# ArielleRosinski/pyGAT

Hardware: AMD Instinct MI355X
Metric: GAT-layer fwd+bwd edges/sec (higher is better)
Workload: dtype f32; 1 GPU; RMAT scale 20 (1048576 nodes, 10760610 edges incl. self loops, max degree 26737), Fin 128, 8 heads x 16, concat+ELU, dropout 0, fwd+bwd (dW, da); nodes=1048576, edges=10760610, fin=128, heads=8, f_out=16, parallelism=single GPU, heads_per_gpu=8, gemm_products=split-bf16, launch=stream launches (pygat_amd.GATLevelFn)

## Files before the change

include/pygat_amd.h:

```cpp
#ifndef PYGAT_AMD_H
#define PYGAT_AMD_H

#include <stdint.h>
#include <stddef.h>

#ifdef __cplusplus
extern "C" {
#endif

#define PYGAT_ABI_VERSION 16

enum {
  PYGAT_OK = 0,
  PYGAT_EINVAL = -1,
  PYGAT_EHIP = -2,
  PYGAT_ENODEV = -3
};

enum {
  PYGAT_F_ELU = 1,
  PYGAT_F_SKIP = 2,
  PYGAT_F_MAIN_ONLY = 4,
  PYGAT_F_FIXUP_ONLY = 8
};
// ... 31 lines not shown
                   const pygat_out_segments* out, int accumulate,
                   int split_k, void* ws, int gemm_mode, void* stream);

typedef struct {
  int w;
  int64_t stride;
} pygat_col_blocks;
int pygat_gemm_f32_blocked(int transA, int transB, int M, int N, int64_t K,
                           const float* A, int64_t lda, const pygat_col_blocks* a_blk, const float* B, int64_t ldb,
                           const pygat_out_segments* out, const pygat_col_blocks* c_blk, int accumulate,
                           int split_k, void* ws, int gemm_mode, void* stream);

int pygat_pack_params(int H, int Fin, int Fo, const float* W, const float* a,
                      const float* w_skip, float* Wcat, int64_t ldw, float* a_pad,
                      void* stream);
#define PYGAT_MAX_HEADS_TABLE 16
int pygat_pack_params_heads(int H, int Fin, int Fo, const float* const* W, const float* const* a,
                            const float* const* w_skip, float* Wcat, int64_t ldw, float* a_pad, void* stream);
int pygat_stack_heads(int H, int64_t nW, int nA, int64_t nS, const float* const* W, const float* const* a,
                      const float* const* w_skip, float* W_out, float* a_out, float* skip_out, void* stream);
int pygat_stack_heads_padded(int H, int64_t nW, int64_t nW_out, int nA, int64_t nS, int64_t nS_out, const float* const* W,
                             const float* const* a, const float* const* w_skip, float* W_out, float* a_out, float* skip_out,
                             void* stream);
int pygat_project(int n, int Fin, int H, int Fo, const float* X, int64_t ldx, const float* Wcat, int64_t ldw, const float* a_pad,
                  float* Wh, float* Sk, float* s, int split_k, void* ws, int gemm_mode, void* stream);
int pygat_project_blocked(int n, int Fin, int H, int Fo, const float* X, int64_t ldx, const pygat_col_blocks* x_blk,
                          const float* Wcat, int64_t ldw, const float* a_pad, float* Wh, float* Sk, float* s, int split_k,
                          void* ws, int gemm_mode, void* stream);
int pygat_attn_scores(int n, int H, int Fo, float* Wh, const float* wh_mask, const float* a_pad,
                      float* s, float* t, void* stream);
int pygat_unpack_wgrad(int H, int Fin, int Fo, const float* dWcat, int64_t ld,
                       int col_offset, float* dW, void* stream);

typedef struct {
  int n;
  int64_t nnz;
  const int32_t* rowptr;
  const int32_t* edge_rc;
  int slot_edges;
  const int32_t* slot_begin;
  const int32_t* cut_rows;
  int n_cut;
  int n_cut_wide;
  int64_t slot_first;
  int64_t slot_count;
  const int32_t* slot_meta;
  const int32_t* slot_order;
  const int32_t* user_row;
} pygat_graph;

int pygat_edge_pairs(int n, const int32_t* rowptr, const int32_t* col, int32_t* edge_rc, void* stream);

int pygat_slot_bounds(int n, int64_t nnz, const int32_t* rowptr, const int32_t* edge_rc, int slot_edges,
                      int32_t* slot_begin, void* stream);
int pygat_slot_meta(int n, int64_t nnz, const int32_t* rowptr, const int32_t* edge_rc, int slot_edges,
                    const int32_t* slot_begin, int32_t* slot_meta, void* stream);

size_t pygat_partials_bytes(int64_t nnz, int slot_edges, int H, int Fp);

int pygat_head_group(int n, int H, int Fo);

int pygat_gat_forward_phases_ok(int n, int H, int Fo);
int pygat_gat_forward(const pygat_graph* g, int H, int Fo, float alpha, int flags,
                      const float* Wh, const float* s, const float* a_pad, const float* sk,
                      const float* att_mask,
                      float* out, float* hattn, float* m, float* Z, float* aneg, float* qneg,
                      void* part, void* stream);

int pygat_head_mean(int n, int H, int Fo, const float* hattn, const float* sk,
                    float* out, void* stream);

int pygat_gat_backward_prepare(int n, int H, int Fo, int flags, int mean_mode,
                               const float* G, const float* y, const float* sk,
                               const float* s, const float* m, const float* Z,
                               float* GR, const float* aneg, const float* qneg, float alpha, float* ds,
                               int h_first, int h_count, int head_group, const int32_t* user_row, void* stream);
int pygat_gat_backward_row(const pygat_graph* g, int H, int Fo, float alpha,
                           const float* Wh, const float* a_pad, const float* GR,
                           const float* att_mask, float* ds, void* part, int h_first, int h_count, int head_group,
                           void* stream);
size_t pygat_gat_backward_col_da_bytes(const pygat_graph* gT, int H, int Fo, int head_group);
// ... 154 lines not shown
```

pygat_amd/_lib.py:

```python
from __future__ import annotations

import ctypes as C
import os

import torch

_HERE = os.path.dirname(os.path.abspath(__file__))
LIB_PATH = os.path.join(_HERE, "libpygat_amd.so")
from .config import config as _config
if _config.lib_path:
    LIB_PATH = os.path.abspath(_config.lib_path)

ABI_VERSION = 16
F_ELU = 1
F_SKIP = 2
F_MAIN_ONLY = 4
F_FIXUP_ONLY = 8

SYMBOLS = [
    "pygat_abi_version", "pygat_last_error", "pygat_padded_width", "pygat_device_count",
    "pygat_device_name", "pygat_kernel_footprint", "pygat_default_gemm_mode", "pygat_dense_row_counts", "pygat_scan_workspace_bytes",
    "pygat_exclusive_scan_i32", "pygat_dense_fill_cols", "pygat_csr_symmetric_perm",
    "pygat_gemm_workspace_bytes", "pygat_gemm_f32", "pygat_gemm_f32_blocked", "pygat_project_blocked", "pygat_wgrad_blocked", "pygat_pack_params", "pygat_pack_params_heads", "pygat_stack_heads", "pygat_stack_heads_padded", "pygat_project", "pygat_attn_scores",
    "pygat_unpack_wgrad",
# ... 1 lines not shown
    "pygat_gat_backward_prepare", "pygat_gat_backward_row", "pygat_gat_backward_col", "pygat_gat_backward_rowsum",
    "pygat_gat_backward_col_da_bytes", "pygat_a_grad_fold",
    "pygat_gat_backward_col_phases_ok", "pygat_gat_backward_col_phase", "pygat_gat_backward_col_finish",
    "pygat_agrad_workspace_bytes", "pygat_a_grad", "pygat_wgrad_workspace_bytes", "pygat_wgrad",
    "pygat_gatv2_forward", "pygat_gatv2_backward_prepare", "pygat_gatv2_workspace_bytes", "pygat_gatv2_backward",
    "pygat_gat_attention", "pygat_gatv2_attention",
    "pygat_alpha_grad_rows", "pygat_alpha_grad_cols", "pygat_alpha_grad_apply",
    "pygat_gat_edge_workspace_bytes", "pygat_gat_edge_forward", "pygat_gat_edge_alpha", "pygat_gat_edge_backward_rows",
    "pygat_gat_edge_backward_cols",
    "pygat_gat_bf16_workspace_bytes", "pygat_gat_pack_bf16", "pygat_gat_forward_bf16",
    "pygat_spmm_workspace_bytes", "pygat_spmm_forward", "pygat_spmm_grad_values",
    "pygat_dropout_mask", "pygat_dropout_mask2", "pygat_dropout_expand", "pygat_dropout_head_sum", "pygat_pack_blockdiag",
    "pygat_unpack_blockdiag",
    "pygat_headmask_supported", "pygat_dropout_bits", "pygat_project_dropout_workspace_bytes", "pygat_project_dropout",
    "pygat_wgrad_dropout_workspace_bytes",
    "pygat_wgrad_dropout", "pygat_dropout_head_sum_bits",
    "pygat_nll_workspace_bytes", "pygat_elu_logsoftmax_nll", "pygat_elu_logsoftmax_nll_backward",
    "pygat_project_sparse", "pygat_wgrad_sparse", "pygat_wgrad_sparse_workspace_bytes", "pygat_dropout_narrow", "pygat_dx_dropout", "pygat_adam_step", "pygat_bce_workspace_bytes", "pygat_bce_with_logits", "pygat_bce_with_logits_backward",
]

MAX_ADAM_TENSORS = 48
MAX_SEGMENTS = 4


class OutSegments(C.Structure):
    _fields_ = [("nseg", C.c_int), ("col_start", C.c_int32 * (MAX_SEGMENTS + 1)), ("ptr", C.c_void_p * MAX_SEGMENTS),
                ("ld", C.c_int64 * MAX_SEGMENTS)]


class ColBlocks(C.Structure):
    _fields_ = [("w", C.c_int), ("stride", C.c_int64)]


class Graph(C.Structure):
    _fields_ = [("n", C.c_int), ("nnz", C.c_int64), ("rowptr", C.c_void_p), ("edge_rc", C.c_void_p),
                ("slot_edges", C.c_int), ("slot_begin", C.c_void_p), ("cut_rows", C.c_void_p),
                ("n_cut", C.c_int), ("n_cut_wide", C.c_int), ("slot_first", C.c_int64), ("slot_count", C.c_int64),
                ("slot_meta", C.c_void_p), ("slot_order", C.c_void_p), ("user_row", C.c_void_p)]


def _load():
    if not os.path.exists(LIB_PATH):
        raise ImportError(
            f"pygat_amd: {LIB_PATH} not found. Build it with `python -c 'import __graft_entry__ as g; "
            f"g.build()'` or `make -C pygat_amd/csrc`. There is no CPU/PyTorch fallback for the hot path.")
    lib = C.CDLL(LIB_PATH)
    missing = [s for s in SYMBOLS if not hasattr(lib, s)]
    if missing:
        raise ImportError(f"pygat_amd: {LIB_PATH} lacks symbols {missing}")
    p, i, i64, f, sz = C.c_void_p, C.c_int, C.c_int64, C.c_float, C.c_size_t
    lib.pygat_abi_version.restype = i
    lib.pygat_last_error.restype = C.c_char_p
    lib.pygat_padded_width.argtypes = [i]
    lib.pygat_device_name.argtypes = [C.c_char_p, i]
    lib.pygat_kernel_footprint.argtypes = [C.c_char_p, C.POINTER(C.c_int), C.POINTER(C.c_int)]
    lib.pygat_default_gemm_mode.argtypes = []
    lib.pygat_dense_row_counts.argtypes = [p, i, i64, i, p, p]
    lib.pygat_scan_workspace_bytes.argtypes = [i64]
    lib.pygat_scan_workspace_bytes.restype = sz
    lib.pygat_exclusive_scan_i32.argtypes = [p, i64, p, p, p]
    lib.pygat_dense_fill_cols.argtypes = [p, i, i64, i, p, p, p]
    lib.pygat_csr_symmetric_perm.argtypes = [i, p, p, p, p, p]
    lib.pygat_gemm_workspace_bytes.argtypes = [i, i, i]
    lib.pygat_gemm_workspace_bytes.restype = sz
    lib.pygat_gemm_f32.argtypes = [i, i, i, i, i64, p, i64, p, i64, C.POINTER(OutSegments), i, i, p, i, p]
    CB = C.POINTER(ColBlocks)
    lib.pygat_gemm_f32_blocked.argtypes = [i, i, i, i, i64, p, i64, CB, p, i64, C.POINTER(OutSegments), CB, i, i, p, i, p]
    lib.pygat_project_blocked.argtypes = [i, i, i, i, p, i64, CB, p, i64, p, p, p, p, i, p, i, p]
    lib.pygat_wgrad_blocked.argtypes = [i, i, i, i, p, i64, CB, p, p, p, p, i, p, i, i, i, p]
    lib.pygat_pack_params.argtypes = [i, i, i, p, p, p, p, i64, p, p]
    lib.pygat_pack_params_heads.argtypes = [i, i, i, p, p, p, p, i64, p, p]
# ... 132 lines not shown
```

pygat_amd/csrc/core.hip:

```cpp
#include "common.h"
#include <string.h>

namespace pygat {
static thread_local char g_err[512] = "";

void set_error(const char* fmt, ...) {
  va_list ap;
  va_start(ap, fmt);
  vsnprintf(g_err, sizeof(g_err), fmt, ap);
  va_end(ap);
}

static const int g_default_split = [] { const char* e = getenv("PYGAT_GEMM_F32"); return (e && atoi(e) != 0) ? 0 : 1; }();
bool gemm_split(int mode) { return mode == PYGAT_GEMM_DEFAULT ? g_default_split != 0 : mode == PYGAT_GEMM_SPLIT_BF16; }
}

extern "C" int pygat_default_gemm_mode(void) { return pygat::g_default_split ? PYGAT_GEMM_SPLIT_BF16 : PYGAT_GEMM_FP32_MFMA; }

extern "C" int pygat_abi_version(void) { return PYGAT_ABI_VERSION; }
extern "C" const char* pygat_last_error(void) { return pygat::g_err; }
extern "C" int pygat_padded_width(int f_out) { return pygat::padded_width(f_out); }

namespace pygat {
int footprint_k2_headline(int* regs, int* scratch);
int footprint_k4_headline_da(int* regs, int* scratch);
int footprint_gemm_x3(int which, int* regs, int* scratch);
int footprint_k14(int which, int* regs, int* scratch);
int footprint_k15(const char* name, int* regs, int* scratch);
int footprint_k16(const char* name, int* regs, int* scratch);
int footprint_k17(const char* name, int* regs, int* scratch);
}

extern "C" int pygat_kernel_footprint(const char* kernel, int* num_regs, int* scratch_bytes) {
  PYGAT_REQUIRE(kernel && num_regs && scratch_bytes, "kernel_footprint: null argument");
  if (!strcmp(kernel, "k2_headline")) return pygat::footprint_k2_headline(num_regs, scratch_bytes);
  if (!strcmp(kernel, "k4_headline_da")) return pygat::footprint_k4_headline_da(num_regs, scratch_bytes);
  if (!strcmp(kernel, "tn_x3w")) return pygat::footprint_gemm_x3(0, num_regs, scratch_bytes);
  if (!strcmp(kernel, "x3gw")) return pygat::footprint_gemm_x3(1, num_regs, scratch_bytes);
  if (!strcmp(kernel, "k1_x3_tail")) return pygat::footprint_gemm_x3(2, num_regs, scratch_bytes);
  static const char* const k14[] = {"k14_rows_long", "k14_cols_long", "k14_rows_wave", "k14_cols_wave", "k14_apply"};
  for (int w = 0; w < 5; ++w)
    if (!strcmp(kernel, k14[w])) return pygat::footprint_k14(w, num_regs, scratch_bytes);
  if (!strncmp(kernel, "k15_", 4)) return pygat::footprint_k15(kernel, num_regs, scratch_bytes);
  if (!strncmp(kernel, "k16_", 4)) return pygat::footprint_k16(kernel, num_regs, scratch_bytes);
  if (!strncmp(kernel, "k17_", 4)) return pygat::footprint_k17(kernel, num_regs, scratch_bytes);
  pygat::set_error("kernel_footprint: unknown kernel '%s' (k2_headline, k4_headline_da, tn_x3w, x3gw, k1_x3_tail, k14_rows_long, "
                   "k14_cols_long, k14_rows_wave, k14_cols_wave, k14_apply)", kernel);
  return PYGAT_EINVAL;
}

extern "C" int pygat_device_count(void) {
  int n = 0;
  if (hipGetDeviceCount(&n) != hipSuccess) {
    (void)hipGetLastError();
    return 0;
  }
  return n;
}

extern "C" int pygat_device_name(char* host_buf, int len) {
  if (!host_buf || len <= 0) return PYGAT_EINVAL;
  int dev = 0;
  hipDeviceProp_t p;
  if (hipGetDevice(&dev) != hipSuccess || hipGetDeviceProperties(&p, dev) != hipSuccess) {
    (void)hipGetLastError();
    pygat::set_error("no HIP device");
    return PYGAT_ENODEV;
  }
  snprintf(host_buf, (size_t)len, "%s (%s)", p.name, p.gcnArchName);
  return PYGAT_OK;
}
```

pygat_amd/csrc/k2_forward.hip:

```cpp
#include "attn_common.h"

namespace pygat {

struct FwdArgs {
  GraphDev g;
  RowShape rs;
  float alpha;
  int flags;
  const float* Wh;
  int64_t ldwh;
  const float* s;
  const float* a_pad;
  const float* sk;
  const float* mask;
  float* out;
  float* hattn;
  float* m;
  float* Z;
  float* part;
  float* aneg;
  float* qneg;
};

__device__ __forceinline__ float lrelu(float z, float alpha) { return z > 0.f ? z : alpha * z; }

template <bool AUX>
__device__ __forceinline__ void fold_edge(float& m, float& z, float4& a, float& zn, float4& an, float ev, bool neg,
                                          float4 w, float mk) {
  const float d = ev - m;
  const float ex = __expf(-fabsf(d));
  const bool up = d > 0.f;
  const float sc = up ? ex : 1.f, p = up ? 1.f : ex;
  z = fmaf(z, sc, p);
  const float pm = p * mk;
  a.x = fmaf(a.x, sc, pm * w.x); a.y = fmaf(a.y, sc, pm * w.y);
  a.z = fmaf(a.z, sc, pm * w.z); a.w = fmaf(a.w, sc, pm * w.w);
  if constexpr (AUX) {
    const float pn = neg ? p : 0.f, pmn = neg ? pm : 0.f;
    zn = fmaf(zn, sc, pn);
    an.x = fmaf(an.x, sc, pmn * w.x); an.y = fmaf(an.y, sc, pmn * w.y);
    an.z = fmaf(an.z, sc, pmn * w.z); an.w = fmaf(an.w, sc, pmn * w.w);
  }
  m = up ? ev : m;
}

template <bool AUX>
__device__ __forceinline__ void merge_state(float& m, float& z, float4& a, float& zn, float4& an, float m2, float z2,
                                            float4 a2, float zn2, float4 an2) {
  const float mn = fmaxf(m, m2);
  const float sa = __expf(m - mn), sb = __expf(m2 - mn);
  z = z * sa + z2 * sb;
  a.x = a.x * sa + a2.x * sb; a.y = a.y * sa + a2.y * sb;
  a.z = a.z * sa + a2.z * sb; a.w = a.w * sa + a2.w * sb;
  if constexpr (AUX) {
// ... 82 lines not shown
    st4(p + lc.cofs[v], st.acc[v]);
    if constexpr (AUX) st4(p + R + 2 * H + lc.cofs[v], st.accn[v]);
    if (((lc.cofs[v] >> 2) & (a.rs.lph - 1)) == 0) {
      p[R + lc.head[v]] = st.m[v];
      p[R + H + lc.head[v]] = st.z[v];
      if constexpr (AUX) p[2 * R + 2 * H + lc.head[v]] = st.zn[v];
    }
  }
}
template <int VEC, bool AUX>
struct PartRec {
  float m[VEC], z[VEC];
  float4 acc[VEC];
  float zn[AUX ? VEC : 1];
  float4 accn[AUX ? VEC : 1];
};
template <int VEC, bool AUX>
__device__ __forceinline__ void part_load(const FwdArgs& a, const LaneCols<VEC>& lc, const float* p, PartRec<VEC, AUX>& r) {
  const int R = a.rs.R, H = a.rs.H;
#pragma unroll
  for (int v = 0; v < VEC; ++v) {
    r.m[v] = p[R + lc.head[v]]; r.z[v] = p[R + H + lc.head[v]]; r.acc[v] = ld4(p + lc.cofs[v]);
    if constexpr (AUX) { r.zn[v] = p[2 * R + 2 * H + lc.head[v]]; r.accn[v] = ld4(p + R + 2 * H + lc.cofs[v]); }
  }
}
template <int VEC, bool AUX>
__device__ __forceinline__ void part_merge(RowState<VEC, AUX>& st, const PartRec<VEC, AUX>& r) {
#pragma unroll
  for (int v = 0; v < VEC; ++v)
    merge_state<AUX>(st.m[v], st.z[v], st.acc[v], st.zn[AUX ? v : 0], st.accn[AUX ? v : 0], r.m[v], r.z[v], r.acc[v],
                     r.zn[AUX ? v : 0], r.accn[AUX ? v : 0]);
}

template <int LPR, int VEC, bool AUX, int LPH = 0, int CR = 0>
__device__ __forceinline__ void fwd_flush(const FwdArgs& a, const LaneCols<VEC>& lc, int64_t k, int i,
                                          bool is_head, bool is_tail, const RowState<VEC, AUX>& st) {
  if (is_head || is_tail) {
    part_store<VEC, AUX>(a, lc, a.part + (2 * k + (is_head ? 0 : 1)) * part_stride<AUX>(a.rs), st);
  } else {
    fwd_finish<LPR, VEC, AUX, LPH, CR>(a, lc, i, st);
  }
}

#ifndef PYGAT_K2_PREFETCH_ALL
#define PYGAT_K2_PREFETCH_ALL 0
#endif
#ifndef PYGAT_K2_PREFETCH_TRAIN
#define PYGAT_K2_PREFETCH_TRAIN 1
#endif
#ifndef PYGAT_K2_HEADLINE_WAVES
#define PYGAT_K2_HEADLINE_WAVES 4
#endif
#ifndef PYGAT_K2_NARROW_U
#define PYGAT_K2_NARROW_U 4
#endif
template <int LPR, int VEC, bool V2, bool AUX, bool FAST, int LPH = 0, int CR = 0>
__global__ __launch_bounds__(256) __attribute__((amdgpu_waves_per_eu((AUX && FAST && VEC == 1 && LPR > 8) ? PYGAT_K2_HEADLINE_WAVES : 1))) void gat_fwd_kernel(FwdArgs a) {
  constexpr int EPW = 64 / LPR;
  constexpr bool NARROW = (VEC == 1 && LPR <= 8);
  constexpr bool PREF = NARROW || (PYGAT_K2_PREFETCH_ALL && VEC == 1) || (PYGAT_K2_PREFETCH_TRAIN && AUX && FAST && VEC == 1);
  constexpr int U = (VEC == 1) ? (NARROW ? PYGAT_K2_NARROW_U : 4) : 2;
  const int lane = threadIdx.x & 63;
  const int64_t kl = ((int64_t)blockIdx.x * (blockDim.x >> 6) + (threadIdx.x >> 6)) * EPW + lane / LPR;
  if (kl >= a.g.kn) return;
  const int64_t k = a.g.order ? a.g.order[kl] : a.g.k0 + kl;
  int64_t e0, e1;
  const int2* __restrict__ rc = a.g.rc;
  int r_first;
  bool head_partial, tail_known = false, tail_flag = false;
  if (a.g.meta) {
    const int4 mt = a.g.meta[k];
    e0 = mt.x; e1 = mt.y; r_first = mt.z;
    head_partial = (mt.w & 1) != 0; tail_known = true; tail_flag = (mt.w & 2) != 0;
  } else {
    slot_range(a.g, k, &e0, &e1);
    r_first = rc[e0].x;
    head_partial = a.g.rowptr[r_first] < e0;
  }
  const LaneCols<VEC> lc = lane_cols<LPR, VEC>(a.rs);
  const int R = CR ? CR : a.rs.R;
  const int64_t ldh = CR ? CR / (4 * (LPH ? LPH : 1)) : a.rs.ldh;

  int cur = r_first;
  const int lph = LPH > 0 ? LPH : (a.rs.lph < 64 ? a.rs.lph : 64);
  float4 adst[VEC];
#pragma unroll
  for (int v = 0; v < VEC; ++v) {
    adst[v] = V2 ? ld4(a.a_pad + (int64_t)lc.head[v] * a.rs.Fp + (lc.cofs[v] & (a.rs.Fp - 1)))
                 : ld4(a.a_pad + (int64_t)lc.head[v] * 2 * a.rs.Fp + a.rs.Fp + (lc.cofs[v] & (a.rs.Fp - 1)));
    if (!lc.valid[v]) adst[v] = make_float4(0.f, 0.f, 0.f, 0.f);
  }
  const int64_t ldw = CR ? CR : a.ldwh;
  RowState<VEC, AUX> st;
  st.reset();

  int2 pn[PREF ? U : 1];
  if constexpr (PREF) {
#pragma unroll
    for (int u = 0; u < U; ++u) pn[u] = rc[(e0 + u < e1) ? e0 + u : e1 - 1];
  }
  for (int64_t e = e0; e < e1; e += U) {
    int2 p[U];
#pragma unroll
    for (int u = 0; u < U; ++u) {
      if constexpr (PREF) p[u] = pn[u];
      else p[u] = rc[(e + u < e1) ? e + u : e1 - 1];
    }
    if constexpr (!PREF) __builtin_amdgcn_sched_barrier(0);
    float sv[U][VEC], tv[U][VEC], mk[U][VEC];
    float4 wv[U][VEC];
// ... 19 lines not shown
        } else {
          sv[u][v] = a.s[(int64_t)p[u].x * ldh + lc.head[v]];
        }
      }
    if constexpr (PREF) {
#pragma unroll
      for (int u = 0; u < U; ++u) pn[u] = rc[(e + U + u < e1) ? e + U + u : e1 - 1];
    }
#pragma unroll
    for (int u = 0; u < U; ++u)
#pragma unroll
      for (int v = 0; v < VEC; ++v) {
        if constexpr (V2) { tv[u][v] = group_sum_rt(sv[u][v], lph); }
        else { tv[u][v] = group_sum_rt(dot4(wv[u][v], adst[v]), lph); }
      }
#pragma unroll
    for (int u = 0; u < U; ++u) {
      if (e + u < e1) {
        if (p[u].x != cur) {
          fwd_flush<LPR, VEC, AUX, LPH, CR>(a, lc, k, cur, cur == r_first && head_partial, false, st);
          cur = p[u].x;
          st.reset();
        }
#pragma unroll
        for (int v = 0; v < VEC; ++v) {
          const float zz = sv[u][v] + tv[u][v];
          fold_edge<AUX>(st.m[v], st.z[v], st.acc[v], st.zn[AUX ? v : 0], st.accn[AUX ? v : 0],
                         V2 ? tv[u][v] : lrelu(zz, a.alpha), !(zz > 0.f), wv[u][v], mk[u][v]);
        }
      }
    }
  }
  const bool tail_partial = tail_known ? tail_flag : a.g.rowptr[cur + 1] > e1;
  fwd_flush<LPR, VEC, AUX, LPH, CR>(a, lc, k, cur, cur == r_first && head_partial, tail_partial, st);
}

template <int LPR, int VEC, bool AUX, int NW, int G = 64 / LPR>
__device__ __forceinline__ void fwd_merge_row(const FwdArgs& a, const LaneCols<VEC>& lc, float* fix_sm, int64_t k, int r,
                                              int npieces, bool wide, int w) {
  constexpr int PF = (VEC == 1) ? 4 : 2;
  const int lane = threadIdx.x & 63, slot = lane / LPR, g = slot % G;
  const int64_t PS = part_stride<AUX>(a.rs);
  RowState<VEC, AUX> st;
  st.reset();
  if (wide || w == 0) {
    const int nw = wide ? NW : 1;
    for (int q = (wide ? w : 0) * G * PF + g; q < npieces; q += nw * G * PF) {
      PartRec<VEC, AUX> rec[PF];
#pragma unroll
      for (int f = 0; f < PF; ++f) {
        const int qq = q + f * G;
        const int qc = qq < npieces ? qq : q;
        part_load<VEC, AUX>(a, lc, a.part + (qc == 0 ? 2 * k + 1 : 2 * (k + qc)) * PS, rec[f]);
      }
#pragma unroll
      for (int f = 0; f < PF; ++f)
        if (q + f * G < npieces) part_merge<VEC, AUX>(st, rec[f]);
    }
#pragma unroll
    for (int off = LPR; off < LPR * G; off <<= 1) {
#pragma unroll
      for (int v = 0; v < VEC; ++v) {
        const float mo = __shfl_xor(st.m[v], off), zo = __shfl_xor(st.z[v], off);
        float4 ao, no = make_float4(0.f, 0.f, 0.f, 0.f);
        float zno = 0.f;
        ao.x = __shfl_xor(st.acc[v].x, off); ao.y = __shfl_xor(st.acc[v].y, off);
        ao.z = __shfl_xor(st.acc[v].z, off); ao.w = __shfl_xor(st.acc[v].w, off);
        if constexpr (AUX) {
          zno = __shfl_xor(st.zn[v], off);
          no.x = __shfl_xor(st.accn[v].x, off); no.y = __shfl_xor(st.accn[v].y, off);
          no.z = __shfl_xor(st.accn[v].z, off); no.w = __shfl_xor(st.accn[v].w, off);
        }
        merge_state<AUX>(st.m[v], st.z[v], st.acc[v], st.zn[AUX ? v : 0], st.accn[AUX ? v : 0], mo, zo, ao, zno, no);
      }
    }
  }
  if (wide) {
    if (slot == 0) part_store<VEC, AUX>(a, lc, fix_sm + w * PS, st);
    __syncthreads();
    if (w == 0 && slot == 0) {
#pragma unroll
      for (int ww = 1; ww < NW; ++ww) {
        PartRec<VEC, AUX> rec;
        part_load<VEC, AUX>(a, lc, fix_sm + ww * PS, rec);
        part_merge<VEC, AUX>(st, rec);
      }
// ... 114 lines not shown
  PYGAT_REQUIRE((aneg == nullptr) == (qneg == nullptr) && (!aneg || (m && !v2 && aligned16(aneg))),
                "gat_forward: aneg and qneg come together, need m/Z, 16-byte alignment and the v1 layer");
  PYGAT_REQUIRE(aligned16(Wh) && aligned16(part) && aligned16(a_pad) && (!sk || aligned16(sk)) && (!hattn || aligned16(hattn)) &&
                    (!out || Fo != Fp || aligned16(out)),
                "gat_forward: row tables must be 16-byte aligned");
  hipStream_t st = (hipStream_t)stream;
  const int64_t nslots = a.g.kn;
  const int hg = v2 ? H : head_group_fwd_n(a.g.n, H, Fp);
  const bool do_main = !(flags & PYGAT_F_FIXUP_ONLY), do_fix = !(flags & PYGAT_F_MAIN_ONLY);
  PYGAT_REQUIRE(do_main || do_fix, "gat_forward: PYGAT_F_MAIN_ONLY and PYGAT_F_FIXUP_ONLY exclude each other");
  PYGAT_REQUIRE((do_main && do_fix) || hg >= H, "gat_forward: a single phase needs the level in one head window (pygat_gat_forward_phases_ok)");
  flags &= ~(PYGAT_F_MAIN_ONLY | PYGAT_F_FIXUP_ONLY);
  for (int h0 = 0; h0 < H; h0 += hg) {
    const int hc = (H - h0 < hg) ? H - h0 : hg;
    PYGAT_REQUIRE(make_window_shape(H, Fo, hc, &a.rs),
                  "gat_forward: unsupported H=%d F'=%d (a pass takes rows of at most 1024 floats)", hc, Fo);
    a.alpha = alpha; a.flags = flags;
    a.Wh = Wh + (int64_t)h0 * Fp; a.ldwh = v2 ? 2 * a.rs.ldr : a.rs.ldr;
    a.s = s ? s + h0 : nullptr;
    a.a_pad = a_pad + (int64_t)h0 * (v2 ? 1 : 2) * Fp;
    a.sk = sk ? sk + (int64_t)h0 * Fp : nullptr;
    a.mask = att_mask ? att_mask + h0 : nullptr;
    a.out = out ? out + (int64_t)h0 * Fo : nullptr;
    a.hattn = hattn ? hattn + (int64_t)h0 * Fp : nullptr;
    a.m = m ? m + h0 : nullptr; a.Z = Z ? Z + h0 : nullptr;
    a.aneg = aneg ? aneg + (int64_t)h0 * Fp : nullptr; a.qneg = qneg ? qneg + h0 : nullptr;
    a.part = (float*)part;
    int lpr, vec;
    pick_lanes(a.rs, &lpr, &vec);
    const unsigned bt = (vec == 1 && lpr <= 8) ? narrow_block() : 256u;
    const unsigned blocks = (unsigned)cdiv(cdiv(nslots, 64 / lpr), bt / 64);
    const bool aux = aneg != nullptr;
    const bool fast = aux && !att_mask && (int64_t)a.g.n * a.ldwh * 4 < ((int64_t)1 << 32);
#define PYGAT_FWD(V2V, AUXV, FASTV)                                                                                   \
    PYGAT_DISPATCH_LANES(lpr, vec, hipLaunchKernelGGL((gat_fwd_kernel<LPR, VEC, V2V, AUXV, FASTV>), dim3(blocks),    \
                                                      dim3(bt), 0, st, a))
    if (!do_main) {}
    else if (v2) PYGAT_FWD(true, false, false);
    else if (aux && fast && lpr == 32 && vec == 1 && a.rs.lph == 4)
      if (a.rs.R == 128 && a.rs.ldr == 128 && a.rs.ldh == 8 && a.rs.ldo == 128 && a.rs.Fo == 16 && a.ldwh == 128 && !(flags & PYGAT_F_SKIP))
        hipLaunchKernelGGL((gat_fwd_kernel<32, 1, false, true, true, 4, 128>), dim3(blocks), dim3(bt), 0, st, a);
      else
        hipLaunchKernelGGL((gat_fwd_kernel<32, 1, false, true, true, 4>), dim3(blocks), dim3(bt), 0, st, a);
    else if (aux && fast) PYGAT_FWD(false, true, true);
    else if (aux) PYGAT_FWD(false, true, false);
    else PYGAT_FWD(false, false, false);
#undef PYGAT_FWD
    PYGAT_CHECK_LAUNCH("gat_forward");
    const bool listed = a.g.cut != nullptr;
    const int fix_waves = listed ? FIX_LIST_WAVES : 4;
    const size_t fix_lds = fix_waves * (size_t)(aux ? part_stride<true>(a.rs) : part_stride<false>(a.rs)) * sizeof(float);
    const unsigned fb = listed ? (unsigned)(a.g.n_cut_wide + cdiv(a.g.n_cut - a.g.n_cut_wide, FIX_LIST_WAVES * fix_rows_per_wave(lpr)))
                               : (unsigned)cdiv(nslots, FIX_SCREEN);
    if ((listed && a.g.n_cut == 0) || !do_fix) continue;
#define PYGAT_FIX(AUXV)                                                                                               \
    do {                                                                                                              \
      if (listed) {                                                                                                   \
        PYGAT_DISPATCH_LANES(lpr, vec, hipLaunchKernelGGL((gat_fwd_fixup_list_kernel<LPR, VEC, AUXV>), dim3(fb),     \
                                                          dim3(64 * FIX_LIST_WAVES), fix_lds, st, a));                \
      } else {                                                                                                        \
        PYGAT_DISPATCH_LANES(lpr, vec, hipLaunchKernelGGL((gat_fwd_fixup_kernel<LPR, VEC, AUXV>), dim3(fb), dim3(256), \
                                                          fix_lds, st, a));                                           \
      }                                                                                                               \
    } while (0)
    if (aux) PYGAT_FIX(true); else PYGAT_FIX(false);
#undef PYGAT_FIX
    PYGAT_CHECK_LAUNCH("gat_forward_fixup");
  }
  return PYGAT_OK;
}

extern "C" int pygat_head_group(int n, int H, int Fo) {
  const int Fp = padded_width(Fo);
  if (n <= 0 || H <= 0 || Fp <= 0) return 0;
  return head_group_bwd(n, H, Fp);
}


static int footprint_of(const void* fn, int* regs, int* scratch) {
  hipFuncAttributes at;
  const hipError_t e = hipFuncGetAttributes(&at, fn);
  if (e != hipSuccess) {
    (void)hipGetLastError();
    pygat::set_error("kernel_footprint: %s", hipGetErrorString(e));
    return PYGAT_EHIP;
  }
  *regs = at.numRegs; *scratch = (int)at.localSizeBytes;
  return PYGAT_OK;
}
namespace pygat {
int footprint_k2_headline(int* regs, int* scratch) {
  return footprint_of(reinterpret_cast<const void*>(&gat_fwd_kernel<32, 1, false, true, true, 4, 128>), regs, scratch);
}
}

extern "C" int pygat_gat_forward_phases_ok(int n, int H, int Fo) {
  const int Fp = padded_width(Fo);
  if (n <= 0 || H <= 0 || Fp <= 0) return 0;
  return head_group_fwd_n(n, H, Fp) >= H ? 1 : 0;
}

extern "C" int pygat_gat_forward(const pygat_graph* g, int H, int Fo, float alpha, int flags, const float* Wh,
                                 const float* s, const float* a_pad, const float* sk, const float* att_mask,
                                 float* out, float* hattn, float* m, float* Z, float* aneg, float* qneg, void* part,
                                 void* stream) {
  return launch_forward(g, H, Fo, alpha, flags, Wh, 0, s, a_pad, sk, att_mask, out, hattn, m, Z, aneg, qneg, part, stream);
}

extern "C" int pygat_gatv2_forward(const pygat_graph* g, int H, int Fo, float alpha, int flags, const float* WW,
                                   const float* a2, const float* sk, const float* att_mask, float* out,
                                   float* hattn, float* m, float* Z, void* part, void* stream) {
  return launch_forward(g, H, Fo, alpha, flags, WW, 1, nullptr, a2, sk, att_mask, out, hattn, m, Z, nullptr, nullptr, part, stream);
}

extern "C" int pygat_head_mean(int n, int H, int Fo, const float* hattn, const float* sk, float* out,
                               void* stream) {
  int Fp = padded_width(Fo);
  PYGAT_REQUIRE(n > 0 && H > 0 && Fp > 0 && hattn && out, "head_mean: bad arguments");
  hipLaunchKernelGGL(head_mean_kernel, dim3((unsigned)cdiv((int64_t)n * Fo, 256)), dim3(256), 0,
                     (hipStream_t)stream, n, H, Fo, Fp, hattn, sk, out);
  PYGAT_CHECK_LAUNCH("head_mean");
  return PYGAT_OK;
}
```

pygat_amd/graph.py:

```python
from __future__ import annotations

import ctypes as C
import weakref
from typing import Optional, Tuple

import torch

from . import _lib
from ._lib import lib, check
from .config import config as _config

SLOT_ORDER_FN = None
FORCED_SLOT_EDGES = _config.slot_edges
USE_SLOT_META = _config.slot_meta

DEFAULT_SLOT_EDGES = 64


def auto_slot_edges(nnz: int) -> int:
    if FORCED_SLOT_EDGES:
        return int(FORCED_SLOT_EDGES)
    ts = DEFAULT_SLOT_EDGES
    while ts > 4 and nnz // ts < 8192:
        ts //= 2
# ... 7 lines not shown
def _stream() -> int:
    return torch.cuda.current_stream().cuda_stream


def _ptr(t: Optional[torch.Tensor]) -> Optional[int]:
    return None if t is None else t.data_ptr()


class _Pattern:

    def __init__(self, rowptr: torch.Tensor, col: torch.Tensor, slot_edges: int, user_row: Optional[torch.Tensor] = None):
        self.rowptr, self.col, self.slot_edges = rowptr, col, slot_edges
        self.user_row = user_row
        self.n = rowptr.numel() - 1
        self.nnz = col.numel()
        self.edge_rc = torch.empty(self.nnz, 2, dtype=torch.int32, device=rowptr.device)
        with torch.cuda.device(rowptr.device):
            check(lib.pygat_edge_pairs(self.n, rowptr.data_ptr(), col.data_ptr(), self.edge_rc.data_ptr(), _stream()),
                  "edge_pairs")
        self._alt = {}
        self.struct = self._make(slot_edges, True)

    def _make(self, slot_edges: int, snapped: bool):
        key = (slot_edges, snapped)
        if key not in self._alt:
            sb = None
            if snapped:
                nslots = -(-self.nnz // slot_edges)
                sb = torch.empty(nslots + 1, dtype=torch.int32, device=self.rowptr.device)
                with torch.cuda.device(self.rowptr.device):
                    check(lib.pygat_slot_bounds(self.n, self.nnz, self.rowptr.data_ptr(), self.edge_rc.data_ptr(),
                                                slot_edges, sb.data_ptr(), _stream()), "slot_bounds")
            cut, n_cut, n_wide = None, 0, 0
            if snapped:
                sbl = sb.long()
                e0, e1 = sbl[:-1], sbl[1:]
                r_last = self.edge_rc[e1 - 1, 0].long()
                rp = self.rowptr.long()
                row_end = rp[r_last + 1]
                k = torch.nonzero((row_end > e1) & (rp[r_last] >= e0)).flatten()
                if k.numel():
                    k_e = torch.searchsorted(sbl, row_end[k] - 1, right=True) - 1
                    pieces = k_e - k + 1
                    order = torch.argsort(pieces, descending=True, stable=True)
                    cut = torch.stack([k, r_last[k], pieces], 1)[order].to(torch.int32).contiguous()
                    n_cut, n_wide = int(k.numel()), int((pieces > 32).sum().item())
                else:
                    cut = torch.zeros(1, 3, dtype=torch.int32, device=self.rowptr.device)
            meta = torch.empty(-(-self.nnz // slot_edges), 4, dtype=torch.int32, device=self.rowptr.device)
            with torch.cuda.device(self.rowptr.device):
                check(lib.pygat_slot_meta(self.n, self.nnz, self.rowptr.data_ptr(), self.edge_rc.data_ptr(), slot_edges, _ptr(sb),
                                          meta.data_ptr(), _stream()), "slot_meta")
            if not USE_SLOT_META:
                meta = None
            order = SLOT_ORDER_FN(self, meta) if (SLOT_ORDER_FN is not None and meta is not None) else None
            st = _lib.Graph(self.n, self.nnz, _ptr(self.rowptr), _ptr(self.edge_rc), slot_edges, _ptr(sb), _ptr(cut),
                            n_cut, n_wide, 0, 0, _ptr(meta), _ptr(order), _ptr(self.user_row))
            self._alt[key] = (st, sb, cut, meta, order)
        return self._alt[key][0]

    def row_chunks(self, nchunks: int, slot_edges: Optional[int] = None, nslots: Optional[int] = None, row_end: Optional[int] = None):
        ts = slot_edges or self.slot_edges
        key = ("chunks", ts, nchunks, nslots)
        if key not in self._alt:
            base = self._make(ts, True)
            _, sb, cut, meta, _order = self._alt[(ts, True)]
            all_slots = sb.numel() - 1
            nslots = all_slots if nslots is None else int(nslots)
            sbl, rp = sb.long(), self.rowptr.long()
            first_row = self.edge_rc[sbl[:-1], 0].long()
            starts_row = rp[first_row] == sbl[:-1]
            ok = torch.nonzero(starts_row[:nslots]).flatten()
            borders = [0]
            for c in range(1, nchunks):
                tgt = c * nslots // nchunks
                j = int(torch.searchsorted(ok, torch.tensor(tgt, device=ok.device)))
                if j < ok.numel() and int(ok[j]) > borders[-1]:
                    borders.append(int(ok[j]))
            borders.append(nslots)
            out, keep = [], []
            for b0, b1 in zip(borders[:-1], borders[1:]):
                r0 = int(first_row[b0])
                r1 = int(first_row[b1]) if b1 < nslots else (self.n if (row_end is None or nslots == all_slots) else int(row_end))
                sub, n_cut, n_wide = None, 0, 0
                if cut is not None:
                    sel = (cut[:, 0] >= b0) & (cut[:, 0] < b1)
                    sub = cut[sel].contiguous()
                    n_cut, n_wide = int(sub.shape[0]), int((sub[:, 2] > 32).sum().item()) if sub.numel() else 0
                    if n_cut == 0:
                        sub = cut[:1].contiguous()
                st = _lib.Graph(self.n, self.nnz, _ptr(self.rowptr), _ptr(self.edge_rc), ts, _ptr(sb), _ptr(sub), n_cut,
# ... 268 lines not shown
```

Before: 4.061 billion edges/s.

## Merge row-split slot partials inside the work-group via LDS before fixup

Rows that span several edge slots within one forward work-group now combine their partial softmax/accumulator records in shared memory, and a per-work-group cut-row list is built on the host. The global fixup pass then only has to merge across work-groups, with fewer partial records written and read. When a slot order is in use, a separate group-merge kernel does the same combining instead. The cost is extra LDS per block, a __syncthreads, serial merging by the tail lane, and more complex bookkeeping of partial kinds.

```diff
diff --git a/include/pygat_amd.h b/include/pygat_amd.h
--- a/include/pygat_amd.h
+++ b/include/pygat_amd.h
@@ -87,6 +87,7 @@
 int pygat_unpack_wgrad(int H, int Fin, int Fo, const float* dWcat, int64_t ld,
                        int col_offset, float* dW, void* stream);
 
+#define PYGAT_WG_CUT_LISTS 5
 typedef struct {
   int n;
   int64_t nnz;
@@ -102,6 +103,9 @@
   const int32_t* slot_meta;
   const int32_t* slot_order;
   const int32_t* user_row;
+  const int32_t* wg_cut_rows[PYGAT_WG_CUT_LISTS];
+  int wg_n_cut[PYGAT_WG_CUT_LISTS];
+  int wg_n_cut_wide[PYGAT_WG_CUT_LISTS];
 } pygat_graph;
 
 int pygat_edge_pairs(int n, const int32_t* rowptr, const int32_t* col, int32_t* edge_rc, void* stream);
diff --git a/pygat_amd/_lib.py b/pygat_amd/_lib.py
--- a/pygat_amd/_lib.py
+++ b/pygat_amd/_lib.py
@@ -57,11 +57,15 @@
     _fields_ = [("w", C.c_int), ("stride", C.c_int64)]
 
 
+WG_CUT_LISTS = 5
+
+
 class Graph(C.Structure):
     _fields_ = [("n", C.c_int), ("nnz", C.c_int64), ("rowptr", C.c_void_p), ("edge_rc", C.c_void_p),
                 ("slot_edges", C.c_int), ("slot_begin", C.c_void_p), ("cut_rows", C.c_void_p),
                 ("n_cut", C.c_int), ("n_cut_wide", C.c_int), ("slot_first", C.c_int64), ("slot_count", C.c_int64),
-                ("slot_meta", C.c_void_p), ("slot_order", C.c_void_p), ("user_row", C.c_void_p)]
+                ("slot_meta", C.c_void_p), ("slot_order", C.c_void_p), ("user_row", C.c_void_p),
+                ("wg_cut_rows", C.c_void_p * WG_CUT_LISTS), ("wg_n_cut", C.c_int * WG_CUT_LISTS), ("wg_n_cut_wide", C.c_int * WG_CUT_LISTS)]
 
 
 def _load():
diff --git a/pygat_amd/csrc/core.hip b/pygat_amd/csrc/core.hip
--- a/pygat_amd/csrc/core.hip
+++ b/pygat_amd/csrc/core.hip
@@ -23,6 +23,7 @@
 
 namespace pygat {
 int footprint_k2_headline(int* regs, int* scratch);
+int footprint_k2_headline_per_slot(int* regs, int* scratch);
 int footprint_k4_headline_da(int* regs, int* scratch);
 int footprint_gemm_x3(int which, int* regs, int* scratch);
 int footprint_k14(int which, int* regs, int* scratch);
@@ -34,6 +35,7 @@
 extern "C" int pygat_kernel_footprint(const char* kernel, int* num_regs, int* scratch_bytes) {
   PYGAT_REQUIRE(kernel && num_regs && scratch_bytes, "kernel_footprint: null argument");
   if (!strcmp(kernel, "k2_headline")) return pygat::footprint_k2_headline(num_regs, scratch_bytes);
+  if (!strcmp(kernel, "k2_headline_per_slot")) return pygat::footprint_k2_headline_per_slot(num_regs, scratch_bytes);
   if (!strcmp(kernel, "k4_headline_da")) return pygat::footprint_k4_headline_da(num_regs, scratch_bytes);
   if (!strcmp(kernel, "tn_x3w")) return pygat::footprint_gemm_x3(0, num_regs, scratch_bytes);
   if (!strcmp(kernel, "x3gw")) return pygat::footprint_gemm_x3(1, num_regs, scratch_bytes);
@@ -44,7 +46,7 @@
   if (!strncmp(kernel, "k15_", 4)) return pygat::footprint_k15(kernel, num_regs, scratch_bytes);
   if (!strncmp(kernel, "k16_", 4)) return pygat::footprint_k16(kernel, num_regs, scratch_bytes);
   if (!strncmp(kernel, "k17_", 4)) return pygat::footprint_k17(kernel, num_regs, scratch_bytes);
-  pygat::set_error("kernel_footprint: unknown kernel '%s' (k2_headline, k4_headline_da, tn_x3w, x3gw, k1_x3_tail, k14_rows_long, "
+  pygat::set_error("kernel_footprint: unknown kernel '%s' (k2_headline, k2_headline_per_slot, k4_headline_da, tn_x3w, x3gw, k1_x3_tail, k14_rows_long, "
                    "k14_cols_long, k14_rows_wave, k14_cols_wave, k14_apply)", kernel);
   return PYGAT_EINVAL;
 }
diff --git a/pygat_amd/csrc/k2_forward.hip b/pygat_amd/csrc/k2_forward.hip
--- a/pygat_amd/csrc/k2_forward.hip
+++ b/pygat_amd/csrc/k2_forward.hip
@@ -20,6 +20,7 @@
   float* part;
   float* aneg;
   float* qneg;
+  int gsh;
 };
 
 __device__ __forceinline__ float lrelu(float z, float alpha) { return z > 0.f ? z : alpha * z; }
@@ -168,6 +169,31 @@
                      r.zn[AUX ? v : 0], r.accn[AUX ? v : 0]);
 }
 
+template <int VEC, bool AUX>
+__device__ __forceinline__ void part_merge_seq(RowState<VEC, AUX>& st, const PartRec<VEC, AUX>& r) {
+#pragma unroll
+  for (int v = 0; v < VEC; ++v) {
+    const float mn = fmaxf(st.m[v], r.m[v]);
+    const float sa = __expf(st.m[v] - mn), sb = __expf(r.m[v] - mn);
+    st.z[v] = fmaf(st.z[v], sa, __fmul_rn(r.z[v], sb));
+    st.acc[v].x = fmaf(st.acc[v].x, sa, __fmul_rn(r.acc[v].x, sb)); st.acc[v].y = fmaf(st.acc[v].y, sa, __fmul_rn(r.acc[v].y, sb));
+    st.acc[v].z = fmaf(st.acc[v].z, sa, __fmul_rn(r.acc[v].z, sb)); st.acc[v].w = fmaf(st.acc[v].w, sa, __fmul_rn(r.acc[v].w, sb));
+    if constexpr (AUX) {
+      st.zn[v] = fmaf(st.zn[v], sa, __fmul_rn(r.zn[v], sb));
+      st.accn[v].x = fmaf(st.accn[v].x, sa, __fmul_rn(r.accn[v].x, sb)); st.accn[v].y = fmaf(st.accn[v].y, sa, __fmul_rn(r.accn[v].y, sb));
+      st.accn[v].z = fmaf(st.accn[v].z, sa, __fmul_rn(r.accn[v].z, sb)); st.accn[v].w = fmaf(st.accn[v].w, sa, __fmul_rn(r.accn[v].w, sb));
+    }
+    st.m[v] = mn;
+  }
+}
+enum : int {
+  PK_IDLE = -1,
+  PK_NONE = 0,
+  PK_HEAD = 1,
+  PK_TAIL = 2,
+  PK_MID = 3
+};
+
 template <int LPR, int VEC, bool AUX, int LPH = 0, int CR = 0>
 __device__ __forceinline__ void fwd_flush(const FwdArgs& a, const LaneCols<VEC>& lc, int64_t k, int i,
                                           bool is_head, bool is_tail, const RowState<VEC, AUX>& st) {
@@ -190,16 +216,22 @@
 #ifndef PYGAT_K2_NARROW_U
 #define PYGAT_K2_NARROW_U 4
 #endif
-template <int LPR, int VEC, bool V2, bool AUX, bool FAST, int LPH = 0, int CR = 0>
+#ifndef PYGAT_K2_WG_MERGE
+#define PYGAT_K2_WG_MERGE 1
+#endif
+template <int LPR, int VEC, bool V2, bool AUX, bool FAST, int LPH = 0, int CR = 0, bool MERGE = false>
 __global__ __launch_bounds__(256) __attribute__((amdgpu_waves_per_eu((AUX && FAST && VEC == 1 && LPR > 8) ? PYGAT_K2_HEADLINE_WAVES : 1))) void gat_fwd_kernel(FwdArgs a) {
+  static_assert(!MERGE || (VEC == 1 && !V2), "the in-work-group merge is built for one chunk per lane and the v1 scoring");
   constexpr int EPW = 64 / LPR;
   constexpr bool NARROW = (VEC == 1 && LPR <= 8);
   constexpr bool PREF = NARROW || (PYGAT_K2_PREFETCH_ALL && VEC == 1) || (PYGAT_K2_PREFETCH_TRAIN && AUX && FAST && VEC == 1);
   constexpr int U = (VEC == 1) ? (NARROW ? PYGAT_K2_NARROW_U : 4) : 2;
   const int lane = threadIdx.x & 63;
   const int64_t kl = ((int64_t)blockIdx.x * (blockDim.x >> 6) + (threadIdx.x >> 6)) * EPW + lane / LPR;
-  if (kl >= a.g.kn) return;
-  const int64_t k = a.g.order ? a.g.order[kl] : a.g.k0 + kl;
+  if constexpr (!MERGE) {
+    if (kl >= a.g.kn) return;
+  }
+  const int64_t k = (MERGE && kl >= a.g.kn) ? a.g.k0 : (a.g.order ? a.g.order[kl] : a.g.k0 + kl);
   int64_t e0, e1;
   const int2* __restrict__ rc = a.g.rc;
   int r_first;
@@ -212,6 +244,9 @@
     slot_range(a.g, k, &e0, &e1);
     r_first = rc[e0].x;
     head_partial = a.g.rowptr[r_first] < e0;
+  }
+  if constexpr (MERGE) {
+    if (kl >= a.g.kn) e0 = e1;
   }
   const LaneCols<VEC> lc = lane_cols<LPR, VEC>(a.rs);
   const int R = CR ? CR : a.rs.R;
@@ -297,7 +332,71 @@
     }
   }
   const bool tail_partial = tail_known ? tail_flag : a.g.rowptr[cur + 1] > e1;
-  fwd_flush<LPR, VEC, AUX, LPH, CR>(a, lc, k, cur, cur == r_first && head_partial, tail_partial, st);
+  if constexpr (!MERGE) {
+    fwd_flush<LPR, VEC, AUX, LPH, CR>(a, lc, k, cur, cur == r_first && head_partial, tail_partial, st);
+  } else {
+    extern __shared__ __attribute__((aligned(16))) float wg_sm[];
+    const int S = (int)(blockDim.x >> 6) * EPW, j = (int)(threadIdx.x >> 6) * EPW + lane / LPR;
+    const int64_t PS = part_stride<AUX>(a.rs), PSL = (PS + 3) & ~(int64_t)3;
+    int* kinds = reinterpret_cast<int*>(wg_sm + S * PSL);
+    const bool hp = cur == r_first && head_partial;
+    const int kind = kl >= a.g.kn ? PK_IDLE : (tail_partial ? (hp ? PK_MID : PK_TAIL) : (hp ? PK_HEAD : PK_NONE));
+    if (kind == PK_MID && j > 0) part_store<VEC, AUX>(a, lc, wg_sm + j * PSL, st);
+    if (kind == PK_HEAD) part_store<VEC, AUX>(a, lc, a.part + 2 * k * PS, st);
+    if ((lane & (LPR - 1)) == 0) kinds[j] = kind;
+    __syncthreads();
+    if (kind == PK_NONE) {
+      fwd_finish<LPR, VEC, AUX, LPH, CR>(a, lc, cur, st);
+    } else if (kind == PK_TAIL || (kind == PK_MID && j == 0)) {
+      bool ended = false;
+      for (int jj = j + 1; jj < S && kl + (jj - j) < a.g.kn && !ended; ++jj) {
+        PartRec<VEC, AUX> rec;
+        if (kinds[jj] == PK_MID) {
+          part_load<VEC, AUX>(a, lc, wg_sm + jj * PSL, rec);
+        } else {
+          part_load<VEC, AUX>(a, lc, a.part + 2 * (k + (jj - j)) * PS, rec);
+          ended = true;
+        }
+        part_merge_seq<VEC, AUX>(st, rec);
+      }
+      if (ended && kind == PK_TAIL) fwd_finish<LPR, VEC, AUX, LPH, CR>(a, lc, cur, st);
+      else part_store<VEC, AUX>(a, lc, a.part + (2 * k + (kind == PK_TAIL ? 1 : 0)) * PS, st);
+    }
+  }
+}
+
+template <int LPR, bool AUX, int LPH = 0, int CR = 0>
+__global__ __launch_bounds__(256) void gat_fwd_group_merge_kernel(FwdArgs a) {
+  constexpr int EPW = 64 / LPR;
+  const int lane = threadIdx.x & 63;
+  const int64_t kl = ((int64_t)blockIdx.x * (blockDim.x >> 6) + (threadIdx.x >> 6)) * EPW + lane / LPR;
+  if (kl >= a.g.kn) return;
+  const int S = 1 << a.gsh, j = (int)(kl & (S - 1));
+  const int64_t k = a.g.k0 + kl, PS = part_stride<AUX>(a.rs);
+  const int2* __restrict__ rc = a.g.rc;
+  const int4 mt = a.g.meta[k];
+  const bool mid = (mt.w & 3) == 3 && rc[mt.y - 1].x == mt.z;
+  const bool tail = (mt.w & 2) != 0 && !mid;
+  if (!(tail || (mid && j == 0))) return;
+  const LaneCols<1> lc = lane_cols<LPR, 1>(a.rs);
+  RowState<1, AUX> st;
+  {
+    PartRec<1, AUX> own;
+    part_load<1, AUX>(a, lc, a.part + (2 * k + (tail ? 1 : 0)) * PS, own);
+    st.m[0] = own.m[0]; st.z[0] = own.z[0]; st.acc[0] = own.acc[0];
+    if constexpr (AUX) { st.zn[0] = own.zn[0]; st.accn[0] = own.accn[0]; }
+    else { st.zn[0] = 0.f; st.accn[0] = make_float4(0.f, 0.f, 0.f, 0.f); }
+  }
+  bool ended = false;
+  for (int jj = j + 1; jj < S && kl + (jj - j) < a.g.kn && !ended; ++jj) {
+    const int4 m2 = a.g.meta[k + (jj - j)];
+    ended = !((m2.w & 3) == 3 && rc[m2.y - 1].x == m2.z);
+    PartRec<1, AUX> rec;
+    part_load<1, AUX>(a, lc, a.part + 2 * (k + (jj - j)) * PS, rec);
+    part_merge_seq<1, AUX>(st, rec);
+  }
+  if (ended && tail) fwd_finish<LPR, 1, AUX, LPH, CR>(a, lc, rc[mt.y - 1].x, st);
+  else part_store<1, AUX>(a, lc, a.part + (2 * k + (tail ? 1 : 0)) * PS, st);
 }
 
 template <int LPR, int VEC, bool AUX, int NW, int G = 64 / LPR>
@@ -316,7 +415,7 @@
       for (int f = 0; f < PF; ++f) {
         const int qq = q + f * G;
         const int qc = qq < npieces ? qq : q;
-        part_load<VEC, AUX>(a, lc, a.part + (qc == 0 ? 2 * k + 1 : 2 * (k + qc)) * PS, rec[f]);
+        part_load<VEC, AUX>(a, lc, a.part + (qc == 0 ? 2 * k + 1 : 2 * (((k >> a.gsh) + qc) << a.gsh)) * PS, rec[f]);
       }
 #pragma unroll
       for (int f = 0; f < PF; ++f)
@@ -497,21 +596,54 @@
     const unsigned blocks = (unsigned)cdiv(cdiv(nslots, 64 / lpr), bt / 64);
     const bool aux = aneg != nullptr;
     const bool fast = aux && !att_mask && (int64_t)a.g.n * a.ldwh * 4 < ((int64_t)1 << 32);
-#define PYGAT_FWD(V2V, AUXV, FASTV)                                                                                   \
-    PYGAT_DISPATCH_LANES(lpr, vec, hipLaunchKernelGGL((gat_fwd_kernel<LPR, VEC, V2V, AUXV, FASTV>), dim3(blocks),    \
-                                                      dim3(bt), 0, st, a))
+    a.gsh = 0;
+    const int wg_slots = (int)(bt / 64) * (64 / lpr), wg_i = ilog2(wg_slots) - 2;
+    const bool grouped = PYGAT_K2_WG_MERGE && !v2 && vec == 1 && hg >= H && a.g.meta && a.g.k0 == 0 && wg_i >= 0 &&
+                         wg_i < PYGAT_WG_CUT_LISTS && g->wg_cut_rows[wg_i] != nullptr;
+    if (grouped) {
+      PYGAT_REQUIRE(g->wg_n_cut[wg_i] >= 0 && g->wg_n_cut_wide[wg_i] >= 0 && g->wg_n_cut_wide[wg_i] <= g->wg_n_cut[wg_i],
+                    "graph: bad per-work-group cut-row list (n_cut=%d n_cut_wide=%d)", g->wg_n_cut[wg_i], g->wg_n_cut_wide[wg_i]);
+      a.gsh = wg_i + 2;
+      a.g.cut = g->wg_cut_rows[wg_i]; a.g.n_cut = g->wg_n_cut[wg_i]; a.g.n_cut_wide = g->wg_n_cut_wide[wg_i];
+    }
+    const bool merge = grouped && !a.g.order;
+    const size_t ps_f = (size_t)(aux ? part_stride<true>(a.rs) : part_stride<false>(a.rs));
+    const size_t wg_lds = merge ? (size_t)wg_slots * (((ps_f + 3) & ~(size_t)3) + 1) * sizeof(float) : 0;
+#define PYGAT_FWD(V2V, AUXV, FASTV, MV)                                                                               \
+    PYGAT_DISPATCH_LANES(lpr, vec, hipLaunchKernelGGL((gat_fwd_kernel<LPR, VEC, V2V, AUXV, FASTV, 0, 0, (MV && VEC == 1)>), \
+                                                      dim3(blocks), dim3(bt), wg_lds, st, a))
+#define PYGAT_FWD_M(V2V, AUXV, FASTV) do { if (merge) PYGAT_FWD(V2V, AUXV, FASTV, true); else PYGAT_FWD(V2V, AUXV, FASTV, false); } while (0)
+    const bool head8 = aux && fast && lpr == 32 && vec == 1 && a.rs.lph == 4;
+    const bool head8c = head8 && a.rs.R == 128 && a.rs.ldr == 128 && a.rs.ldh == 8 && a.rs.ldo == 128 && a.rs.Fo == 16 && a.ldwh == 128 &&
+                        !(flags & PYGAT_F_SKIP);
     if (!do_main) {}
-    else if (v2) PYGAT_FWD(true, false, false);
-    else if (aux && fast && lpr == 32 && vec == 1 && a.rs.lph == 4)
-      if (a.rs.R == 128 && a.rs.ldr == 128 && a.rs.ldh == 8 && a.rs.ldo == 128 && a.rs.Fo == 16 && a.ldwh == 128 && !(flags & PYGAT_F_SKIP))
-        hipLaunchKernelGGL((gat_fwd_kernel<32, 1, false, true, true, 4, 128>), dim3(blocks), dim3(bt), 0, st, a);
-      else
-        hipLaunchKernelGGL((gat_fwd_kernel<32, 1, false, true, true, 4>), dim3(blocks), dim3(bt), 0, st, a);
-    else if (aux && fast) PYGAT_FWD(false, true, true);
-    else if (aux) PYGAT_FWD(false, true, false);
-    else PYGAT_FWD(false, false, false);
+    else if (v2) PYGAT_FWD(true, false, false, false);
+    else if (head8c && merge)
+      hipLaunchKernelGGL((gat_fwd_kernel<32, 1, false, true, true, 4, 128, true>), dim3(blocks), dim3(bt), wg_lds, st, a);
+    else if (head8c)
+      hipLaunchKernelGGL((gat_fwd_kernel<32, 1, false, true, true, 4, 128>), dim3(blocks), dim3(bt), 0, st, a);
+    else if (head8 && merge)
+      hipLaunchKernelGGL((gat_fwd_kernel<32, 1, false, true, true, 4, 0, true>), dim3(blocks), dim3(bt), wg_lds, st, a);
+    else if (head8)
+      hipLaunchKernelGGL((gat_fwd_kernel<32, 1, false, true, true, 4>), dim3(blocks), dim3(bt), 0, st, a);
+    else if (aux && fast) PYGAT_FWD_M(false, true, true);
+    else if (aux) PYGAT_FWD_M(false, true, false);
+    else PYGAT_FWD_M(false, false, false);
+#undef PYGAT_FWD_M
 #undef PYGAT_FWD
     PYGAT_CHECK_LAUNCH("gat_forward");
+    if (grouped && !merge && do_fix) {
+      const unsigned gb = (unsigned)cdiv(cdiv(nslots, 64 / lpr), 4);
+#define PYGAT_GM(AUXV)                                                                                                \
+      do {                                                                                                            \
+        if (head8c) hipLaunchKernelGGL((gat_fwd_group_merge_kernel<32, AUXV, 4, 128>), dim3(gb), dim3(256), 0, st, a); \
+        else if (head8) hipLaunchKernelGGL((gat_fwd_group_merge_kernel<32, AUXV, 4, 0>), dim3(gb), dim3(256), 0, st, a); \
+        else PYGAT_DISPATCH_LANES(lpr, 1, { (void)VEC; hipLaunchKernelGGL((gat_fwd_group_merge_kernel<LPR, AUXV>), dim3(gb), dim3(256), 0, st, a); }); \
+      } while (0)
+      if (aux) PYGAT_GM(true); else PYGAT_GM(false);
+#undef PYGAT_GM
+      PYGAT_CHECK_LAUNCH("gat_forward_group_merge");
+    }
     const bool listed = a.g.cut != nullptr;
     const int fix_waves = listed ? FIX_LIST_WAVES : 4;
     const size_t fix_lds = fix_waves * (size_t)(aux ? part_stride<true>(a.rs) : part_stride<false>(a.rs)) * sizeof(float);
@@ -555,6 +687,9 @@
 }
 namespace pygat {
 int footprint_k2_headline(int* regs, int* scratch) {
+  return footprint_of(reinterpret_cast<const void*>(&gat_fwd_kernel<32, 1, false, true, true, 4, 128, PYGAT_K2_WG_MERGE != 0>), regs, scratch);
+}
+int footprint_k2_headline_per_slot(int* regs, int* scratch) {
   return footprint_of(reinterpret_cast<const void*>(&gat_fwd_kernel<32, 1, false, true, true, 4, 128>), regs, scratch);
 }
 }
diff --git a/pygat_amd/graph.py b/pygat_amd/graph.py
--- a/pygat_amd/graph.py
+++ b/pygat_amd/graph.py
@@ -63,6 +63,7 @@
                     check(lib.pygat_slot_bounds(self.n, self.nnz, self.rowptr.data_ptr(), self.edge_rc.data_ptr(),
                                                 slot_edges, sb.data_ptr(), _stream()), "slot_bounds")
             cut, n_cut, n_wide = None, 0, 0
+            wg = []
             if snapped:
                 sbl = sb.long()
                 e0, e1 = sbl[:-1], sbl[1:]
@@ -76,8 +77,19 @@
                     order = torch.argsort(pieces, descending=True, stable=True)
                     cut = torch.stack([k, r_last[k], pieces], 1)[order].to(torch.int32).contiguous()
                     n_cut, n_wide = int(k.numel()), int((pieces > 32).sum().item())
+                    recs = [torch.div(k_e, 4 << i, rounding_mode="floor") - torch.div(k, 4 << i, rounding_mode="floor") + 1
+                            for i in range(_lib.WG_CUT_LISTS)]
+                    counts = torch.stack([torch.stack([(r > 1).sum(), (r > 32).sum()]) for r in recs]).tolist()
+                    for r, (n_g, n_gw) in zip(recs, counts):
+                        if n_g:
+                            sel = torch.nonzero(r > 1).flatten()
+                            o = torch.argsort(r[sel], descending=True, stable=True)
+                            wg.append((torch.stack([k[sel], r_last[k][sel], r[sel]], 1)[o].to(torch.int32).contiguous(), int(n_g), int(n_gw)))
+                        else:
+                            wg.append((torch.zeros(1, 3, dtype=torch.int32, device=self.rowptr.device), 0, 0))
                 else:
                     cut = torch.zeros(1, 3, dtype=torch.int32, device=self.rowptr.device)
+                    wg = [(cut, 0, 0)] * _lib.WG_CUT_LISTS
             meta = torch.empty(-(-self.nnz // slot_edges), 4, dtype=torch.int32, device=self.rowptr.device)
             with torch.cuda.device(self.rowptr.device):
                 check(lib.pygat_slot_meta(self.n, self.nnz, self.rowptr.data_ptr(), self.edge_rc.data_ptr(), slot_edges, _ptr(sb),
@@ -87,7 +99,11 @@
             order = SLOT_ORDER_FN(self, meta) if (SLOT_ORDER_FN is not None and meta is not None) else None
             st = _lib.Graph(self.n, self.nnz, _ptr(self.rowptr), _ptr(self.edge_rc), slot_edges, _ptr(sb), _ptr(cut),
                             n_cut, n_wide, 0, 0, _ptr(meta), _ptr(order), _ptr(self.user_row))
+            if meta is not None:
+                for i, (lst, n_g, n_gw) in enumerate(wg):
+                    st.wg_cut_rows[i], st.wg_n_cut[i], st.wg_n_cut_wide[i] = _ptr(lst), n_g, n_gw
             self._alt[key] = (st, sb, cut, meta, order)
+            self._alt[("wg", key)] = wg
         return self._alt[key][0]
 
     def row_chunks(self, nchunks: int, slot_edges: Optional[int] = None, nslots: Optional[int] = None, row_end: Optional[int] = None):
```

Result: no change. 4.053 billion edges/s (-0.2%).
